# MaxHalford/sorobn

Measured on NVIDIA H100. Metric: exact-inference queries/sec, higher is better.
Workload: dtype f32

## Files before the change

### sorobn_b200/csrc/sbn_api.cu

```cuda
#include <cuda_runtime.h>

#include <algorithm>
#include <cmath>
#include <cstdarg>
#include <cstdio>
#include <cstdlib>
#include <cstring>
#include <string>
#include <vector>

#include "sbn_chain.h"
#include "sbn_count.cuh"
#include "sbn_deriv.cuh"
#include "sbn_gibbs.cuh"
#include "sbn_internal.h"
#include "sbn_join.h"
#include "sbn_kernels.cuh"
#include "sbn_launch.h"
#include "sbn_marginal.cuh"
#include "sbn_mpe.cuh"
#include "sbn_pair.h"
#include "sbn_sample.cuh"
#include "sbn_soft.cuh"
#include "sbn_tma.h"
// ... 1160 lines not shown
        sbn_soft_pack<float><<<grid, threads, 0, stream>>>(static_cast<const float *>(in.lik), in.ld_lik, rows, n_soft,
                                                           P->d_soft, P->d_arena, P->ld, P->d_log_max);
    return cudaGetLastError();
}

inline bool hoisted(const sbn_program *P, const StepDesc &st) { return P->mode == 1 && st.kind == 0; }

inline bool chain_on(const sbn_program *P) {
    return P->use_chain && P->chain_fits && P->use_tiled && !P->use_branches && !P->segments.empty();
}

inline bool pair_on(const sbn_program *P) {
    return P->use_pair && P->use_tiled && !P->use_branches && (!chain_on(P) || P->pairs_avoid_segments) && !P->pairs.empty();
}

int run_table_steps(sbn_program *P) {
    if (P->mode != 1) return SBN_OK;
    SbnStep q;
    for (const StepDesc &st : P->steps) {
        if (!hoisted(P, st)) continue;
        build_params(P, st, nullptr, 0, 1, &q);
        SBN_CUDA(launch_step(P, st, q, P->stream));
    }
    SBN_CUDA(cudaStreamSynchronize(P->stream));
    P->setup_launches = P->launches;
    P->launches = 0;
    return SBN_OK;
}

inline bool fold_normalise(const sbn_program *P, const StepDesc &st, const SbnStep &q) {
#if !SBN_FOLD_NORMALISE
    (void)P;
    (void)st;
    (void)q;
    return false;
#endif
    static const bool enabled = [] {
        const char *e = getenv("SOROBN_B200_FOLD_NORMALISE");
        return e ? atoi(e) != 0 : true;
    }();
    return enabled && P->kind == kPosterior && !P->f64 && P->post_batched && st.kind == 1 && q.tile_off != nullptr &&
           q.slab_off == nullptr && st.n_tiles == 1 && st.n_out == P->Q && !sbn_tma_eligible(P, st);
}

int issue_all(sbn_program *P, const uint8_t *d_ev, int64_t ld_ev, int64_t n_rows, float *d_out, int64_t ld_out,
              cudaStream_t stream, cudaEvent_t *events, const RunInputs &in = {}) {
    if (P->kind == kSample) SBN_CUDA(cudaMemsetAsync(in.flags(P), 0, static_cast<size_t>(n_rows), stream));
    if (!P->soft.empty()) SBN_CUDA(launch_soft_pack(P, n_rows, in, stream));
    SbnStep q;
    int k = 0;
    int n_decoded = 0;
    bool folded = false;
    bool skip_second = false;
    for (const StepDesc &st : P->steps) {
        if (events) SBN_CUDA(cudaEventRecord(events[k], stream));
        ++k;
        if (hoisted(P, st)) continue;
        if (in.forward && !P->forward[k - 1]) continue;
        if (st.kind >= 2) {
            const int decoded = st.kind == 4 || st.kind == 5 ? n_decoded++ : 0;
            SBN_CUDA(launch_kind_step(P, st, decoded, d_ev, ld_ev, n_rows, d_out, ld_out, in, stream));
            continue;
        }
        const int seg = chain_on(P) ? P->seg_first[k - 1] : -1;
        if (seg == -2) continue;
        if (seg >= 0) {
            P->launches++;
            SBN_CUDA(sbn_chain_launch(P, *P->segments[seg], d_ev, ld_ev, n_rows, d_out, ld_out, stream));
            continue;
        }
        int pair = pair_on(P) ? P->pair_first[k - 1] : -1;
        if (pair == -2 && !skip_second) pair = -1;
        skip_second = false;
        if (pair == -2) continue;
        if (pair >= 0 && !sbn_pair_fits(P, *P->pairs[pair])) pair = -1;
        if (pair >= 0) {
            skip_second = true;
            P->launches++;
            SBN_CUDA(sbn_pair_launch(P, *P->pairs[pair], d_ev, ld_ev, n_rows, stream));
            continue;
        }
        build_params(P, st, d_ev, ld_ev, n_rows, &q);
        if (k == static_cast<int>(P->steps.size()) && fold_normalise(P, st, q)) {
            q.norm_out = d_out;
            q.norm_ld = ld_out;
            q.norm_totals = P->d_total;
            q.norm_min = SBN_MIN_TOTAL_F32;
            folded = true;
        }
        SBN_CUDA(launch_step(P, st, q, stream));
    }
    if (events) SBN_CUDA(cudaEventRecord(events[k], stream));
    switch (P->kind) {
        case kPosterior:
            if (!folded && !(chain_on(P) && P->segments.back()->ends_in_posterior))
                SBN_CUDA(launch_normalise(P, d_out, ld_out, n_rows, stream));
            break;
        case kCounts:
        case kGrad: SBN_CUDA(launch_prob(P, n_rows, d_out, nullptr, stream)); break;
        case kSample: SBN_CUDA(launch_prob(P, n_rows, d_out, in.flags(P), stream)); break;
        case kJoint: SBN_CUDA(launch_prob(P, n_rows, P->d_total, nullptr, stream)); break;
        case kMarginals:
        case kMpe:
        case kMap: break;
    }
    if (events) SBN_CUDA(cudaEventRecord(events[k + 1], stream));
    return SBN_OK;
}

int issue_branched(sbn_program *P, const uint8_t *d_ev, int64_t ld_ev, int64_t n_rows, float *d_out, int64_t ld_out,
                   cudaStream_t origin, const RunInputs &in) {
    const int n_steps = static_cast<int>(P->steps.size());
    const int n_slots = static_cast<int>(P->slots.size());
    std::vector<int> last_writer(n_slots, -1);
    std::vector<std::vector<int>> readers(n_slots);
    std::vector<int> stream_of(n_steps, 0);
    cudaEvent_t fork = P->step_done[n_steps];
    if (!P->soft.empty()) SBN_CUDA(launch_soft_pack(P, n_rows, in, origin));
    SBN_CUDA(cudaEventRecord(fork, origin));
    bool joined[sbn_program::kBranches] = {false, false, false, false};
    int rr = 0;
    SbnStep q;
    for (int s = 0; s < n_steps; ++s) {
        const StepDesc &st = P->steps[s];
        if (hoisted(P, st)) continue;
        std::vector<int> deps;
        int home = -1;
        int64_t home_size = -1;
// ... 505 lines not shown
    if (n_table_floats > 0) {
        SBN_CUDA_P(cudaMalloc(&P->d_tables, static_cast<size_t>(n_table_floats) * elem));
        SBN_CUDA_P(cudaMemcpyAsync(P->d_tables, tables, static_cast<size_t>(n_table_floats) * elem,
                                   cudaMemcpyHostToDevice, P->stream));
    }
    int64_t shared_floats = 0;
    for (Slot &s : P->slots)
        if (!s.batched) shared_floats += round_up(s.padded, 64);
    if (shared_floats > 0) {
        SBN_CUDA_P(cudaMalloc(&P->d_shared, static_cast<size_t>(shared_floats) * elem));
        SBN_CUDA_P(cudaMemsetAsync(P->d_shared, 0, static_cast<size_t>(shared_floats) * elem, P->stream));
        int64_t off = 0;
        for (Slot &s : P->slots)
            if (!s.batched) {
                s.ptr = reinterpret_cast<float *>(reinterpret_cast<char *>(P->d_shared) + off * elem);
                off += round_up(s.padded, 64);
            }
    }
    {
        std::vector<int32_t> &tile_words = P->h_tile_words;
        tile_words.clear();
        plan_tiles(P, &tile_words);
        if (!tile_words.empty()) {
            SBN_CUDA_P(cudaMalloc(&P->d_tile_off, tile_words.size() * 4));
            SBN_CUDA_P(cudaMemcpyAsync(P->d_tile_off, tile_words.data(), tile_words.size() * 4,
                                       cudaMemcpyHostToDevice, P->stream));
        }
        SBN_CUDA_P(cudaStreamSynchronize(P->stream));
        if (P->kind == kPosterior && P->soft.empty()) sbn_chain_plan(P);
    }
    if (!P->soft.empty()) {
        P->use_tma = false;
        std::vector<int32_t> desc;
        for (const auto &sv : P->soft) {
            int64_t off = 0;
            for (int s = 0; s < sv.first; ++s)
                if (P->slots[s].batched) off += P->slots[s].size;
            desc.push_back(static_cast<int32_t>(off));
            desc.push_back(sv.second);
        }
        SBN_CUDA_P(cudaMalloc(&P->d_soft, desc.size() * 4));
        SBN_CUDA_P(cudaMemcpyAsync(P->d_soft, desc.data(), desc.size() * 4, cudaMemcpyHostToDevice, P->stream));
        SBN_CUDA_P(cudaStreamSynchronize(P->stream));
    }
    {
        static bool done[64] = {false};
        if (device < 64 && !done[device]) {
            SBN_CUDA_P(sbn_batched_set_attrs());
            SBN_CUDA_P(set_tiled_attrs());
            SBN_CUDA_P(sbn_chain_set_attrs());
            SBN_CUDA_P(sbn_tma_set_attrs());
            SBN_CUDA_P(sbn_join_set_attrs());
            SBN_CUDA_P(sbn_triple_rows_set_attrs());
            SBN_CUDA_P(sbn_marginal_set_attrs());
            SBN_CUDA_P(sbn_count_set_attrs());
            SBN_CUDA_P(sbn_deriv_set_attrs());
            SBN_CUDA_P(sbn_joint_set_attrs());
            SBN_CUDA_P(sbn_sample_set_attrs());
            SBN_CUDA_P(sbn_argmax_set_attrs());
            SBN_CUDA_P(sbn_batched_logdomain_set_attrs());
            done[device] = true;
        }
    }
    if (P->kind == kCounts || P->kind == kGrad) {
        for (const StepDesc &st : P->steps)
            if (st.kind == 3)
                P->partial_doubles = std::max<int64_t>(P->partial_doubles, count_grid(P, st, INT32_MAX) * SBN_COUNT_WARPS * st.span);
        SBN_CUDA_P(cudaMalloc(&P->d_counts, static_cast<size_t>(P->n_counts) * 8));
    }
#undef SBN_CUDA_P
    rc = run_table_steps(P);
    if (rc != SBN_OK) return bail(rc);
    {
        cudaError_t e = P->kind == kPosterior ? sbn_pair_plan(P) : cudaSuccess;
        if (e != cudaSuccess) return bail(fail(SBN_E_CUDA, "planning the paired steps failed: %s", cudaGetErrorString(e)));
    }
    *out = P;
    return SBN_OK;
}

int sbn_program_create(int device, const int32_t *words, int64_t n_words, const float *tables, int64_t n_table_floats,
                       sbn_program **out) {
    return create_common(device, words, n_words, tables, n_table_floats, false, out);
}

int sbn_program_create_f64(int device, const int32_t *words, int64_t n_words, const double *tables,
                           int64_t n_table_doubles, sbn_program **out) {
    return create_common(device, words, n_words, tables, n_table_doubles, true, out);
}

void sbn_program_destroy(sbn_program *P) {
    if (!P) return;
    cudaSetDevice(P->device);
    free_scratch(P);
    sbn_chain_free(P);
    sbn_pair_free(P);
    cudaFree(P->d_shared);
    cudaFree(P->d_counts);
    cudaFree(P->d_drawn);
    cudaFree(P->d_sample_args);
    cudaFree(P->d_soft);
    cudaFree(P->d_tile_off);
    cudaFree(P->d_tables);
    if (P->stream) cudaStreamDestroy(P->stream);
    for (auto &b : P->branch)
        if (b) cudaStreamDestroy(b);
// ... 757 lines not shown
```

### sorobn_b200/csrc/sbn_internal.h

```cpp
#pragma once
#include <cuda_runtime.h>
#include <stdint.h>

#include <string>
#include <utility>
#include <vector>

#include "../../include/sorobn_b200.h"

struct EvAxis {
    int col, stride, card;
};
struct InDesc {
    bool is_slot;
    int id;
    bool batched;
    int sx;
    std::vector<EvAxis> ev;
    std::vector<int> estrides;
    std::vector<int> strides;
};
struct StepDesc {
    int kind;
    int out_slot;
    int cx;
    int64_t n_out;
    std::vector<int> cards;
    std::vector<int> ecards;
    int64_t zoff_pos = -1;
    int64_t zoff_tiled_pos = -1;
    std::vector<InDesc> in;
    int tile = 0;
    int nu = 0, na = 0, nb = 0, nc = 0;
    std::vector<int> order;
    int64_t n_tiles = 0;
    int64_t tile_off_pos = 0;
    bool slab = false;
    bool big_tables = false;
    int slab_ma = 0, n_slab = 0;
    int64_t slab_off_pos = 0;
    int64_t slab_tile_off_pos = 0;
    int64_t tiles_per_super = 0, n_super = 0;
    int64_t slice_pos = -1;
    int64_t slice_tpc = 0;
    int64_t slice_smem = 0;
    int64_t q_offset = -1;
    int n_common = 0;
    std::vector<EvAxis> key;
    std::vector<int> cstrides;
    int64_t span = 0;
    int64_t soff_pos = -1, coff_pos = -1;
    bool logsumexp = false;
};
struct Slot {
    bool batched;
    int64_t size;
    int64_t padded;
    float *ptr;
};

inline int64_t round_up(int64_t v, int64_t m) { return (v + m - 1) / m * m; }
// ... 52 lines not shown
    int n_sampled = 0;
    uint8_t *d_drawn = nullptr;
    int64_t drawn_bytes = 0;
    uint32_t *d_sample_args = nullptr;
    std::vector<std::pair<int, int>> soft;
    int n_lik = 0;
    int32_t *d_soft = nullptr;
    void *d_lik = nullptr;
    double *d_log_max = nullptr;
    std::vector<char> forward;
    double *d_weight = nullptr;
    CachedGraph forward_graph;
    std::vector<std::pair<int64_t, int64_t>> tables;
    std::vector<int64_t> table_padded;
    float *d_tables = nullptr;
    std::vector<Slot> slots;
    std::vector<StepDesc> steps;

    int64_t reserved_rows = 0;
    int64_t ld = 0;
    float *d_arena = nullptr;
    float *d_shared = nullptr;
    int32_t *d_tile_off = nullptr;
    float *d_total = nullptr;
    uint8_t *d_ev = nullptr;
    float *d_out = nullptr;
    cudaStream_t stream = nullptr;
    static constexpr int kBranches = 4;
    cudaStream_t branch[kBranches] = {nullptr, nullptr, nullptr, nullptr};
    std::vector<cudaEvent_t> step_done;
    std::vector<cudaEvent_t> pipe_events;
    bool use_branches = false;

    bool use_graph = true;
    bool use_tiled = true;
    bool use_slab = true;
    bool use_preload = true;
    CachedGraph graph;
    CachedGraph pipe_graph;

    int64_t launches = 0;
    int64_t setup_launches = 0;

    std::vector<SbnSegment *> segments;
    std::vector<int> seg_first;
    float *d_chain_scratch = nullptr;
    bool use_chain = true;
    bool use_tma = true;
    bool chain_fits = true;
    std::vector<int32_t> h_tile_words;

    std::vector<SbnPair *> pairs;
    std::vector<int> pair_first;
    float *d_pair_canon = nullptr;
    int32_t *d_pair_tiles = nullptr;
    bool use_pair = true;
    bool pairs_avoid_segments = false;
};
```

### sorobn_b200/csrc/sbn_pair.cu

```cuda
#include "sbn_pair.h"

#include <algorithm>
#include <cstdlib>
#include <cstring>

#include "sbn_internal.h"
#include "sbn_kernels.cuh"
#include "sbn_launch.h"

namespace {

constexpr int kV = 2;

__device__ __forceinline__ void pair_coef8(float (&c)[SBN_PAIR_PW], const float *s) {
    const float4 lo = *reinterpret_cast<const float4 *>(s);
    const float4 hi = *reinterpret_cast<const float4 *>(s + 4);
    c[0] = lo.x, c[1] = lo.y, c[2] = lo.z, c[3] = lo.w;
    c[4] = hi.x, c[5] = hi.y, c[6] = hi.z, c[7] = hi.w;
}

template <int V>
__device__ __forceinline__ void pair_ev_offsets(const SbnPairParams &p, const SbnPairEv &d, int b, int (&e)[V]) {
#pragma unroll
    for (int l = 0; l < V; ++l) e[l] = 0;
// ... 7 lines not shown
struct PairG {
    const float *p;
    uint32_t base;
    uint32_t x[SBN_PAIR_T], d0[SBN_PAIR_T], d1[SBN_PAIR_T];
};

template <int MODE, int V>
__device__ __forceinline__ void pair_step(const float (&in)[SBN_PAIR_T][SBN_PAIR_T][V], float (&acc)[SBN_PAIR_T][SBN_PAIR_T][V],
                                          const float *k, const int (&e)[V], const PairG &G) {
    constexpr int T = SBN_PAIR_T, PW = SBN_PAIR_PW;
    constexpr bool PACKED = V == 2 && (MODE == SBN_PAIR_CE || MODE == SBN_PAIR_GB || MODE == SBN_PAIR_GC);
#pragma unroll
    for (int d0 = 0; d0 < T; ++d0)
#pragma unroll
        for (int d1 = 0; d1 < T; ++d1)
#pragma unroll
            for (int l = 0; l < V; ++l) acc[d0][d1][l] = 0.f;
#pragma unroll
    for (int x = 0; x < T; ++x) {
        float c[V][PW];
        float cp[T][V];
        if constexpr (MODE == SBN_PAIR_B) {
#pragma unroll
            for (int l = 0; l < V; ++l) pair_coef8(c[l], k + e[l] + x * PW);
        } else if constexpr (MODE == SBN_PAIR_GB) {
#pragma unroll
            for (int d1 = 0; d1 < T; ++d1) sbn_ldv<V>(cp[d1], G.p + (G.base + G.x[x] + G.d1[d1]));
        }
#pragma unroll
        for (int d0 = 0; d0 < T; ++d0) {
            if constexpr (MODE == SBN_PAIR_CU) {
                pair_coef8(c[0], k + (x * T + d0) * PW);
            } else if constexpr (MODE == SBN_PAIR_CE) {
#pragma unroll
                for (int d1 = 0; d1 < T; ++d1)
#pragma unroll
                    for (int l = 0; l < V; ++l) cp[d1][l] = k[e[l] + (x * T + d0) * T + d1];
            } else if constexpr (MODE == SBN_PAIR_GC) {
#pragma unroll
                for (int d1 = 0; d1 < T; ++d1) sbn_ldv<V>(cp[d1], G.p + (G.base + G.x[x] + G.d0[d0] + G.d1[d1]));
            }
#pragma unroll
            for (int d1 = 0; d1 < T; ++d1) {
                if constexpr (PACKED) {
                    sbn_fma2(acc[d0][d1], in[x][d0], cp[d1]);
                } else {
#pragma unroll
                    for (int l = 0; l < V; ++l)
                        acc[d0][d1][l] = fmaf(in[x][d0][l], c[MODE == SBN_PAIR_CU ? 0 : l][d1], acc[d0][d1][l]);
                }
            }
        }
    }
}

template <int M1, int M2>
__global__ void __launch_bounds__(SBN_PAIR_ROWS / kV, (M1 >= SBN_PAIR_GB ? 4 : 5)) sbn_pair_kernel(const __grid_constant__ SbnPairParams p) {
    constexpr int T = SBN_PAIR_T, V = kV;
    extern __shared__ __align__(16) float s_canon[];
    __shared__ __align__(8) uint64_t s_bar;
    sbn_pdl_launch_dependents();

    const int rblock = blockIdx.x / p.n_chunks;
    const int chunk = blockIdx.x % p.n_chunks;
    if (threadIdx.x == 0) {
        sbn_mbar_init(&s_bar, 1);
        sbn_fence_mbar_init();
    }
    __syncthreads();
    if (threadIdx.x == 0) {
        sbn_mbar_expect_tx(&s_bar, static_cast<uint32_t>(p.canon_floats) * 4u);
        sbn_tma_bulk_g2s(s_canon, p.canon, static_cast<uint32_t>(p.canon_floats) * 4u, &s_bar);
    }

    const int b = (rblock * static_cast<int>(blockDim.x) + threadIdx.x) * V;
    const bool live = b < p.n_rows;
    int e1[V], e2[V], g1[V], g2[V];
    if (live) {
        pair_ev_offsets<V>(p, p.ev_main1, b, e1);
        pair_ev_offsets<V>(p, p.ev_main2, b, e2);
        pair_ev_offsets<V>(p, p.ev_pre1, b, g1);
        pair_ev_offsets<V>(p, p.ev_pre2, b, g2);
    }
    sbn_mbar_wait(&s_bar, 0);
    if (!live) return;
    sbn_pdl_wait();

    const uint32_t ld = static_cast<uint32_t>(p.ld);
    const float *const fp = p.f + b;
    float *const op = p.out + b;
    uint32_t xs[T], ys[T], ow[T], oz[T];
#pragma unroll
    for (int d = 0; d < T; ++d) {
        xs[d] = static_cast<uint32_t>(min(d, p.cx - 1) * p.f_sx) * ld;
        ys[d] = static_cast<uint32_t>(min(d, p.cy - 1) * p.f_sy) * ld;
        ow[d] = static_cast<uint32_t>(d * p.o_sw) * ld;
        oz[d] = static_cast<uint32_t>(d * p.o_sz) * ld;
    }
    PairG G;
    G.p = p.g + b;
    G.base = 0;
    if constexpr (M1 == SBN_PAIR_GB || M1 == SBN_PAIR_GC) {
#pragma unroll
        for (int d = 0; d < T; ++d) {
            G.x[d] = static_cast<uint32_t>(d * p.g_x) * ld;
            G.d0[d] = static_cast<uint32_t>(d * p.g_y) * ld;
            G.d1[d] = static_cast<uint32_t>(d * p.g_w) * ld;
        }
    }
    const int t_begin = chunk * p.tiles_per_cta;
    const int t_end = min(p.n_tiles, t_begin + p.tiles_per_cta);

    for (int t = t_begin; t < t_end; ++t) {
        const int4 r0 = __ldg(reinterpret_cast<const int4 *>(p.tile_off) + 2 * t);
        const int4 r1 = __ldg(reinterpret_cast<const int4 *>(p.tile_off) + 2 * t + 1);
        const uint32_t ob = static_cast<uint32_t>(r0.x) * ld, fb = static_cast<uint32_t>(r0.y) * ld;

        float f[T][T][V];
#pragma unroll
        for (int x = 0; x < T; ++x)
#pragma unroll
            for (int y = 0; y < T; ++y) sbn_ldv<V>(f[x][y], fp + (fb + xs[x] + ys[y]));
        if (p.has_pre1) {
            const float *const k = s_canon + r1.x;
#pragma unroll
            for (int x = 0; x < T; ++x)
#pragma unroll
                for (int y = 0; y < T; ++y)
#pragma unroll
                    for (int l = 0; l < V; ++l) f[x][y][l] *= k[g1[l] + x * T + y];
        }
        float mid[T][T][V];
        if constexpr (M1 == SBN_PAIR_GB || M1 == SBN_PAIR_GC) G.base = static_cast<uint32_t>(r1.z) * ld;
        pair_step<M1, V>(f, mid, s_canon + r0.z, e1, G);
        if (p.has_pre2) {
            const float *const k = s_canon + r1.y;
#pragma unroll
            for (int y = 0; y < T; ++y)
#pragma unroll
                for (int w = 0; w < T; ++w)
#pragma unroll
                    for (int l = 0; l < V; ++l) mid[y][w][l] *= k[g2[l] + y * T + w];
        }
        float acc[T][T][V];
        pair_step<M2, V>(mid, acc, s_canon + r0.w, e2, G);

#pragma unroll
        for (int z = 0; z < T; ++z)
#pragma unroll
            for (int w = 0; w < T; ++w)
                if (w < p.cw && z < p.cz) sbn_stv<V>(op + (ob + ow[w] + oz[z]), acc[w][z]);
    }
}

template <int MINB>
__global__ void __launch_bounds__(SBN_TRIPLE_THREADS, MINB) sbn_triple_kernel(const __grid_constant__ SbnTripleParams p) {
    constexpr int T = SBN_PAIR_T;
    sbn_pdl_entry();
    const int rblock = blockIdx.x / p.n_chunks;
    const int chunk = blockIdx.x % p.n_chunks;
    const int b = rblock * static_cast<int>(blockDim.x) + threadIdx.x;
    if (b >= p.n_rows) return;
    const uint32_t ld = static_cast<uint32_t>(p.ld);
    const int g = threadIdx.y;
    const float *const ap = p.a + b + static_cast<uint32_t>(g * p.a_g) * ld;
    const float *const bp = p.b + b;
    const float *const cp = p.c + b;
    float *const op = p.out + b + static_cast<uint32_t>(g * p.o_g) * ld;
    uint32_t ak[T], aj[T], bj[T], bs[T], ck[T], cz[T];
#pragma unroll
    for (int d = 0; d < T; ++d) {
        ak[d] = static_cast<uint32_t>(d * p.a_k) * ld, aj[d] = static_cast<uint32_t>(d * p.a_j) * ld;
        bj[d] = static_cast<uint32_t>(d * p.b_j) * ld, bs[d] = static_cast<uint32_t>(d * p.b_s) * ld;
        ck[d] = static_cast<uint32_t>(d * p.c_k) * ld, cz[d] = static_cast<uint32_t>(d * p.c_z) * ld;
    }
    const uint32_t oz = static_cast<uint32_t>(p.o_z) * ld, os = static_cast<uint32_t>(p.o_s) * ld;
    const int t_begin = chunk * p.tiles_per_cta;
    const int t_end = min(p.n_tiles, t_begin + p.tiles_per_cta);
    for (int t = t_begin; t < t_end; ++t) {
        const int4 row = __ldg(reinterpret_cast<const int4 *>(p.tile_off) + t);
        float acc[T][T];
#pragma unroll
        for (int z = 0; z < T; ++z)
#pragma unroll
            for (int s = 0; s < T; ++s) acc[z][s] = 0.f;
#pragma unroll 1
        for (int pp = 0; pp < T; ++pp) {
            float A[T][T], B[T][T], C[T][T];
            const uint32_t a0 = static_cast<uint32_t>(row.y + pp * p.a_p) * ld, b0 = static_cast<uint32_t>(row.z + pp * p.b_p) * ld,
                           c0 = static_cast<uint32_t>(row.w + pp * p.c_p) * ld;
#pragma unroll
            for (int j = 0; j < T; ++j)
#pragma unroll
                for (int s = 0; s < T; ++s) B[j][s] = bp[b0 + bj[j] + bs[s]];
#pragma unroll
            for (int k = 0; k < T; ++k)
#pragma unroll
                for (int j = 0; j < T; ++j) A[k][j] = ap[a0 + ak[k] + aj[j]];
#pragma unroll
            for (int k = 0; k < T; ++k)
#pragma unroll
                for (int z = 0; z < T; ++z) C[k][z] = cp[c0 + ck[k] + cz[z]];
#pragma unroll
            for (int k = 0; k < T; ++k) {
                float n[T];
// ... 252 lines not shown
    for (int k = 0; k < n2; ++k)
        if (k != ks && k != kz && k != kg) r2.push_back(k), n_tiles *= s2.cards[k];
    if (n_tiles >= (1LL << 27)) return nullptr;

    SbnPair *pr = new SbnPair();
    memset(&pr->q, 0, sizeof pr->q);
    memset(&pr->t, 0, sizeof pr->t);
    pr->kind = 1;
    pr->step1 = i1, pr->step2 = i2;
    pr->g_in = -1;
    pr->a_in = ai, pr->b_in = 1 - ai, pr->c_in = 1 - mi;
    pr->tile_off_pos = static_cast<int64_t>(tiles->size());
    SbnTripleParams &q = pr->t;
    q.n_tiles = static_cast<int32_t>(n_tiles);
    q.a_j = A.estrides[0], q.a_k = A.strides[jk], q.a_p = A.strides[jp];
    q.b_j = B.estrides[0], q.b_s = B.strides[to1[ks]], q.b_p = B.strides[jp];
    q.c_k = C.estrides[kk], q.c_p = C.estrides[1 - kk], q.c_z = C.strides[kz];
    int64_t os = 1;
    std::vector<int64_t> os2(n2);
    for (int k = 0; k < n2; ++k) os2[k] = os, os *= s2.cards[k];
    q.o_z = static_cast<int32_t>(os2[kz]);
    q.o_s = static_cast<int32_t>(os2[ks]);
    q.group = kg >= 0 ? T : 1;
    q.o_g = kg >= 0 ? static_cast<int32_t>(os2[kg]) : 0;
    q.a_g = kg >= 0 ? A.strides[to1[kg]] : 0;
    std::vector<int> dig(r2.size(), 0);
    for (int64_t t = 0; t < n_tiles; ++t) {
        int64_t ob = 0, ab = 0, bb = 0, cb = 0;
        for (size_t k = 0; k < r2.size(); ++k) {
            const int ax = r2[k];
            ob += dig[k] * os2[ax];
            cb += static_cast<int64_t>(dig[k]) * C.strides[ax];
            if (to1[ax] >= 0) {
                ab += static_cast<int64_t>(dig[k]) * A.strides[to1[ax]];
                bb += static_cast<int64_t>(dig[k]) * B.strides[to1[ax]];
            }
        }
        tiles->push_back(static_cast<int32_t>(ob));
        tiles->push_back(static_cast<int32_t>(ab));
        tiles->push_back(static_cast<int32_t>(bb));
        tiles->push_back(static_cast<int32_t>(cb));
        for (size_t k = 0; k < dig.size(); ++k) {
            if (++dig[k] < s2.cards[r2[k]]) break;
            dig[k] = 0;
        }
    }
    sbn_triple_rows_plan(q, tiles->data() + pr->tile_off_pos, &pr->rows);
    return pr;
}

}

cudaError_t sbn_pair_set_attrs() {
    return cudaSuccess;
}

void sbn_pair_free(sbn_program *P) {
    for (SbnPair *pr : P->pairs) delete pr;
    P->pairs.clear();
    P->pair_first.clear();
    cudaFree(P->d_pair_canon);
    cudaFree(P->d_pair_tiles);
    P->d_pair_canon = nullptr;
    P->d_pair_tiles = nullptr;
}

cudaError_t sbn_pair_plan(sbn_program *P) {
    constexpr int T = SBN_PAIR_T;
    P->pair_first.assign(P->steps.size(), -1);
    if (P->mode != 1 || P->f64) return cudaSuccess;
    static const int min_card = [] {
        const char *e = getenv("SOROBN_B200_PAIR_MIN_CARD");
        return e ? atoi(e) : 4;
    }();

    static const bool triples_on = [] {
        const char *e = getenv("SOROBN_B200_TRIPLE");
        return e ? atoi(e) != 0 : true;
    }();

    HostTables H;
    std::vector<float> canon;
    std::vector<int32_t> tiles;
    cudaError_t err = cudaSuccess;
    bool fetched = false;

    const int n_steps = static_cast<int>(P->steps.size());
    auto launched = [&](int i) { return P->steps[i].kind != 0; };
    P->pairs_avoid_segments = P->use_chain && !P->segments.empty();
    auto in_segment = [&](int i) { return P->pairs_avoid_segments && P->seg_first[i] != -1; };
    for (int i1 = 0; i1 < n_steps; ++i1) {
        if (!launched(i1) || P->pair_first[i1] != -1) continue;
        int i2 = i1 + 1;
        while (i2 < n_steps && !launched(i2)) ++i2;
        if (i2 >= n_steps) break;
        if (in_segment(i1) || in_segment(i2)) continue;
        const StepDesc &s1 = P->steps[i1], &s2 = P->steps[i2];
        if (triples_on) {
            if (SbnPair *tr = plan_triple(P, i1, i2, &tiles)) {
                P->pair_first[i1] = static_cast<int>(P->pairs.size());
                P->pair_first[i2] = -2;
                P->pairs.push_back(tr);
                continue;
            }
        }
        if (s1.kind != 1 || s2.kind != 1 || s1.ecards.size() != 1 || s2.ecards.size() != 1) continue;
        if (s1.tile == 0 || s2.tile == 0) continue;
        int fi = -1, gi = -1, mi = -1, n_b1 = 0, n_b2 = 0;
        for (int i = 0; i < static_cast<int>(s1.in.size()); ++i)
            if (s1.in[i].batched) gi = fi, fi = i, ++n_b1;
        for (int i = 0; i < static_cast<int>(s2.in.size()); ++i)
            if (s2.in[i].batched) mi = i, ++n_b2;
        if (n_b1 < 1 || n_b1 > 2 || n_b2 != 1) continue;
        const InDesc &M = s2.in[mi];
        if (!M.is_slot || M.id != s1.out_slot || !M.ev.empty()) continue;
        if (n_b1 == 2) {
            if (s1.in.size() != 2) continue;
            const int jy0 = axis_of_stride(s1.cards, M.estrides[0]);
            if (jy0 < 0) continue;
            if (s1.in[fi].strides[jy0] == 0 || (s1.in[gi].strides[jy0] != 0 && P->slots[s1.in[gi].id].size > P->slots[s1.in[fi].id].size))
                std::swap(fi, gi);
            if (!s1.in[gi].is_slot || !s1.in[gi].ev.empty() || s1.in[gi].id == s2.out_slot) continue;
// ... 67 lines not shown
            fill_canon(g2, canon.data() + pr->canon_pos + at_g2);
            q.n_tiles = static_cast<int32_t>(n_tiles);
            q.f_sx = F.estrides[0];
            q.f_sy = F.strides[jy];
            q.cx = cx, q.cy = cy, q.cw = s2.cards[kw], q.cz = s2.cards[kz];
            int64_t os = 1;
            std::vector<int64_t> os2(n2);
            for (int k = 0; k < n2; ++k) os2[k] = os, os *= s2.cards[k];
            q.o_sw = static_cast<int32_t>(os2[kw]);
            q.o_sz = static_cast<int32_t>(os2[kz]);
            if (gi >= 0) q.g_x = s1.in[gi].estrides[0], q.g_y = s1.in[gi].strides[jy], q.g_w = s1.in[gi].strides[jw];
            q.has_pre1 = g1.tabs.empty() ? 0 : 1;
            q.has_pre2 = g2.tabs.empty() ? 0 : 1;
            set_ev(&q.ev_main1, c1);
            set_ev(&q.ev_main2, c2);
            set_ev(&q.ev_pre1, g1);
            set_ev(&q.ev_pre2, g2);
            std::vector<int> dig(r2.size(), 0);
            for (int64_t t = 0; t < n_tiles; ++t) {
                int64_t ob = 0, fb = 0;
                for (size_t k = 0; k < r2.size(); ++k) {
                    ob += dig[k] * os2[r2[k]];
                    fb += static_cast<int64_t>(dig[k]) * F.strides[r1[k]];
                }
                tiles.push_back(static_cast<int32_t>(ob));
                tiles.push_back(static_cast<int32_t>(fb));
                tiles.push_back(static_cast<int32_t>(at_c1 + tile_slab(c1, r1, dig)));
                tiles.push_back(static_cast<int32_t>(at_c2 + tile_slab(c2, r2, dig)));
                tiles.push_back(static_cast<int32_t>(at_g1 + tile_slab(g1, r1, dig)));
                tiles.push_back(static_cast<int32_t>(at_g2 + tile_slab(g2, r2, dig)));
                int64_t gb = 0;
                if (gi >= 0)
                    for (size_t k = 0; k < r1.size(); ++k) gb += static_cast<int64_t>(dig[k]) * s1.in[gi].strides[r1[k]];
                tiles.push_back(static_cast<int32_t>(gb));
                tiles.push_back(0);
                for (size_t k = 0; k < dig.size(); ++k) {
                    if (++dig[k] < s2.cards[r2[k]]) break;
                    dig[k] = 0;
                }
            }
            P->pair_first[i1] = static_cast<int>(P->pairs.size());
            P->pair_first[i2] = -2;
            P->pairs.push_back(pr);
            break;
        }
    }
    if (P->pairs.empty()) return cudaSuccess;
    err = cudaMalloc(&P->d_pair_canon, std::max<size_t>(canon.size(), 4) * 4);
    if (err != cudaSuccess) return err;
    err = cudaMalloc(&P->d_pair_tiles, tiles.size() * 4);
    if (err != cudaSuccess) return err;
    if (!canon.empty()) err = cudaMemcpy(P->d_pair_canon, canon.data(), canon.size() * 4, cudaMemcpyHostToDevice);
    if (err != cudaSuccess) return err;
    return cudaMemcpy(P->d_pair_tiles, tiles.data(), tiles.size() * 4, cudaMemcpyHostToDevice);
}

static cudaError_t triple_launch(sbn_program *P, const SbnPair &pr, int64_t n_rows, cudaStream_t stream) {
    SbnTripleParams q = pr.t;
    const StepDesc &s1 = P->steps[pr.step1], &s2 = P->steps[pr.step2];
    q.a = P->slots[s1.in[pr.a_in].id].ptr;
    q.b = P->slots[s1.in[pr.b_in].id].ptr;
    q.c = P->slots[s2.in[pr.c_in].id].ptr;
    q.out = P->slots[s2.out_slot].ptr;
    q.ld = P->ld;
    q.n_rows = static_cast<int32_t>(n_rows);
    q.tile_off = P->d_pair_tiles + pr.tile_off_pos;
    if (sbn_triple_rows_launch(P, pr.rows, q, stream)) return cudaGetLastError();
    const int rows_per_cta = q.group > 1 ? 32 : 128;
    const int64_t n_rblocks = (n_rows + rows_per_cta - 1) / rows_per_cta;
    static const int64_t tpc_env = [] {
        const char *e = getenv("SOROBN_B200_TRIPLE_TPC");
        return e ? atoll(e) : 1LL;
    }();
    static const int minb = [] {
        const char *e = getenv("SOROBN_B200_TRIPLE_MINB");
        return e ? atoi(e) : 3;
    }();
    const int64_t tpc = std::max<int64_t>(1, std::min<int64_t>(q.n_tiles, tpc_env));
    q.tiles_per_cta = static_cast<int32_t>(tpc);
    q.n_chunks = static_cast<int32_t>((q.n_tiles + tpc - 1) / tpc);
    const int64_t grid = q.n_chunks * n_rblocks;
    if (grid >= (1LL << 31)) return cudaErrorInvalidConfiguration;
    const dim3 g(static_cast<unsigned>(grid)), b(rows_per_cta, q.group);
    if (minb == 3) sbn_launch(sbn_triple_kernel<3>, g, b, 0, stream, q);
    else if (minb == 1) sbn_launch(sbn_triple_kernel<1>, g, b, 0, stream, q);
    else sbn_launch(sbn_triple_kernel<2>, g, b, 0, stream, q);
    return cudaGetLastError();
}

bool sbn_pair_fits(const sbn_program *P, const SbnPair &pr) {
    const StepDesc &s1 = P->steps[pr.step1], &s2 = P->steps[pr.step2];
    int64_t entries = P->slots[s2.out_slot].size;
    for (const InDesc &in : s1.in)
        if (in.batched) entries = std::max(entries, P->slots[in.id].size);
    for (const InDesc &in : s2.in)
        if (in.batched && in.id != s1.out_slot) entries = std::max(entries, P->slots[in.id].size);
    const char *e = getenv("SOROBN_B200_PAIR_IDX_LIMIT");
    const int64_t limit = e ? atoll(e) : (1LL << 31);
    return entries * P->ld < limit;
}

cudaError_t sbn_pair_launch(sbn_program *P, const SbnPair &pr, const uint8_t *d_ev, int64_t ld_ev, int64_t n_rows,
                            cudaStream_t stream) {
    if (pr.kind == 1) return triple_launch(P, pr, n_rows, stream);
    SbnPairParams q = pr.q;
    const StepDesc &s1 = P->steps[pr.step1], &s2 = P->steps[pr.step2];
    q.f = P->slots[s1.in[pr.f_in].id].ptr;
    q.g = pr.g_in >= 0 ? P->slots[s1.in[pr.g_in].id].ptr : q.f;
    q.out = P->slots[s2.out_slot].ptr;
    q.ev = d_ev;
    q.ld_ev = ld_ev;
    q.ld = P->ld;
    q.n_rows = static_cast<int32_t>(n_rows);
    q.canon = P->d_pair_canon + pr.canon_pos;
    q.tile_off = P->d_pair_tiles + pr.tile_off_pos;
    const int64_t n_rblocks = (n_rows + SBN_PAIR_ROWS - 1) / SBN_PAIR_ROWS;
    static const int64_t target_env = [] {
        const char *e = getenv("SOROBN_B200_PAIR_CTAS");
        return e ? atoll(e) : 0LL;
    }();
    const int64_t target = target_env > 0 ? target_env : 8LL * P->n_sms * 6;
    const int64_t chunks = std::max<int64_t>(1, std::min<int64_t>(q.n_tiles, target / std::max<int64_t>(1, n_rblocks)));
    const int64_t tpc = (q.n_tiles + chunks - 1) / chunks;
    q.tiles_per_cta = static_cast<int32_t>(tpc);
    q.n_chunks = static_cast<int32_t>((q.n_tiles + tpc - 1) / tpc);
    const int64_t grid = q.n_chunks * n_rblocks;
    if (grid >= (1LL << 31)) return cudaErrorInvalidConfiguration;
    launch_modes(pr, q, static_cast<unsigned>(grid), static_cast<size_t>(q.canon_floats) * 4, stream);
    return cudaGetLastError();
}
```

### sorobn_b200/csrc/sbn_pair.h

```cpp
#pragma once
#include <cuda_runtime.h>
#include <stdint.h>

#include <vector>

#include "../../include/sorobn_b200.h"

#define SBN_PAIR_T 5
#define SBN_PAIR_PW 8
#define SBN_PAIR_MAX_EV 4
#define SBN_PAIR_ROWS 256
#define SBN_TRIPLE_THREADS 160
#define SBN_PAIR_SMEM_MAX (40 * 1024)

struct SbnPairEv {
    int32_t n;
    int32_t col[SBN_PAIR_MAX_EV], stride[SBN_PAIR_MAX_EV], card[SBN_PAIR_MAX_EV];
};

struct SbnPairParams {
    const float *f;
    float *out;
    const uint8_t *ev;
    const float *canon;
// ... 3 lines not shown
    int32_t canon_floats;
    int32_t n_tiles, tiles_per_cta, n_chunks;
    int32_t f_sx, f_sy;
    int32_t cx, cy, cw, cz;
    int32_t o_sw, o_sz;
    int32_t has_pre1, has_pre2;
    SbnPairEv ev_main1, ev_main2, ev_pre1, ev_pre2;
    const float *g;
    int32_t g_x, g_y, g_w;
};

enum SbnPairMode { SBN_PAIR_B = 0, SBN_PAIR_CU = 1, SBN_PAIR_CE = 2, SBN_PAIR_GB = 3, SBN_PAIR_GC = 4 };

struct SbnTripleParams {
    const float *a, *b, *c;
    float *out;
    const int32_t *tile_off;
    int64_t ld;
    int32_t n_rows;
    int32_t n_tiles, tiles_per_cta, n_chunks;
    int32_t a_p, a_k, a_j;
    int32_t b_p, b_j, b_s;
    int32_t c_p, c_k, c_z;
    int32_t o_z, o_s;
    int32_t group;
    int32_t a_g, o_g;
};

#define SBN_TRIPLE_ROWS_R 16
#define SBN_TRIPLE_ROWS_COMBOS 25
#define SBN_TRIPLE_ROWS_MIN_COMBOS 8
struct SbnTripleRows {
    int ok;
    int n_combos;
    int32_t u_card[3], u_stride[3];
    int32_t u_dig[3][SBN_TRIPLE_ROWS_COMBOS];
    int32_t o_off[SBN_TRIPLE_ROWS_COMBOS];
};

struct SbnPair {
    int kind;
    int step1, step2;
    int f_in;
    int g_in;
    int m1, m2;
    SbnPairParams q;
    SbnTripleParams t;
    SbnTripleRows rows;
    int a_in, b_in, c_in;
    int64_t tile_off_pos;
    int64_t canon_pos;
};

struct sbn_program;
cudaError_t sbn_pair_plan(sbn_program *P);
cudaError_t sbn_pair_launch(sbn_program *P, const SbnPair &pr, const uint8_t *d_ev, int64_t ld_ev, int64_t n_rows,
                            cudaStream_t stream);
bool sbn_pair_fits(const sbn_program *P, const SbnPair &pr);
cudaError_t sbn_pair_set_attrs();
void sbn_pair_free(sbn_program *P);

void sbn_triple_rows_plan(const SbnTripleParams &q, const int32_t *tiles, SbnTripleRows *rows);
bool sbn_triple_rows_launch(const sbn_program *P, const SbnTripleRows &rows, const SbnTripleParams &q, cudaStream_t stream);
cudaError_t sbn_triple_rows_set_attrs();
```

Before: 25.38 million.

## Fuse chains of linked pair steps into one persistent shared-memory kernel

Adds a planner that finds consecutive pair contractions whose intermediate slot is consumed only by the next pair, and a persistent kernel that runs the whole run per 16-row block. The input rows stay in shared memory, are double-buffered with cp.async, and only the final output is written back. Canonical tables and tile offsets are loaded once with bulk TMA. The goal is to remove the global-memory round trips for intermediate slots and the separate launches. The cost is heavy shared-memory use, a per-pair runtime mode switch, and __syncthreads between pairs, which may limit occupancy.

```diff
diff --git a/sorobn_b200/csrc/sbn_api.cu b/sorobn_b200/csrc/sbn_api.cu
--- a/sorobn_b200/csrc/sbn_api.cu
+++ b/sorobn_b200/csrc/sbn_api.cu
@@ -1236,10 +1236,12 @@
     int n_decoded = 0;
     bool folded = false;
     bool skip_second = false;
+    int run_last = -1;
     for (const StepDesc &st : P->steps) {
         if (events) SBN_CUDA(cudaEventRecord(events[k], stream));
         ++k;
         if (hoisted(P, st)) continue;
+        if (k - 1 <= run_last) continue;
         if (in.forward && !P->forward[k - 1]) continue;
         if (st.kind >= 2) {
             const int decoded = st.kind == 4 || st.kind == 5 ? n_decoded++ : 0;
@@ -1258,6 +1260,13 @@
         skip_second = false;
         if (pair == -2) continue;
         if (pair >= 0 && !sbn_pair_fits(P, *P->pairs[pair])) pair = -1;
+        const int run = pair >= 0 ? sbn_pair_run_at(P, pair, n_rows) : -1;
+        if (run >= 0) {
+            run_last = P->pair_runs[run].last_step;
+            P->launches++;
+            SBN_CUDA(sbn_pair_run_launch(P, P->pair_runs[run], d_ev, ld_ev, n_rows, stream));
+            continue;
+        }
         if (pair >= 0) {
             skip_second = true;
             P->launches++;
@@ -1869,6 +1878,7 @@
             SBN_CUDA_P(sbn_tma_set_attrs());
             SBN_CUDA_P(sbn_join_set_attrs());
             SBN_CUDA_P(sbn_triple_rows_set_attrs());
+            SBN_CUDA_P(sbn_pair_set_attrs());
             SBN_CUDA_P(sbn_marginal_set_attrs());
             SBN_CUDA_P(sbn_count_set_attrs());
             SBN_CUDA_P(sbn_deriv_set_attrs());
diff --git a/sorobn_b200/csrc/sbn_internal.h b/sorobn_b200/csrc/sbn_internal.h
--- a/sorobn_b200/csrc/sbn_internal.h
+++ b/sorobn_b200/csrc/sbn_internal.h
@@ -7,6 +7,7 @@
 #include <vector>
 
 #include "../../include/sorobn_b200.h"
+#include "sbn_pair.h"
 
 struct EvAxis {
     int col, stride, card;
@@ -165,6 +166,8 @@
 
     std::vector<SbnPair *> pairs;
     std::vector<int> pair_first;
+    std::vector<SbnPairRun> pair_runs;
+    std::vector<int> pair_run_of;
     float *d_pair_canon = nullptr;
     int32_t *d_pair_tiles = nullptr;
     bool use_pair = true;
diff --git a/sorobn_b200/csrc/sbn_pair.cu b/sorobn_b200/csrc/sbn_pair.cu
--- a/sorobn_b200/csrc/sbn_pair.cu
+++ b/sorobn_b200/csrc/sbn_pair.cu
@@ -83,6 +83,63 @@
             }
         }
     }
+}
+
+struct PairIo {
+    const float *fp;
+    float *op;
+    uint32_t fb, ob;
+    uint32_t xs[SBN_PAIR_T], ys[SBN_PAIR_T];
+    uint32_t ow[SBN_PAIR_T], oz[SBN_PAIR_T];
+};
+
+template <int M1, int M2, int V, bool SHARED>
+__device__ __forceinline__ void pair_tile(const SbnPairParams &p, const float *s_canon, const int4 r0, const int4 r1,
+                                          const PairIo &io, PairG &G, uint32_t g_ld, const int (&e1)[V], const int (&e2)[V],
+                                          const int (&g1)[V], const int (&g2)[V]) {
+    constexpr int T = SBN_PAIR_T;
+    float f[T][T][V];
+#pragma unroll
+    for (int x = 0; x < T; ++x)
+#pragma unroll
+        for (int y = 0; y < T; ++y) sbn_ldv<V>(f[x][y], io.fp + (io.fb + io.xs[x] + io.ys[y]));
+    if constexpr (SHARED) __syncthreads();
+    if (p.has_pre1) {
+        const float *const k = s_canon + r1.x;
+#pragma unroll
+        for (int x = 0; x < T; ++x)
+#pragma unroll
+            for (int y = 0; y < T; ++y)
+#pragma unroll
+                for (int l = 0; l < V; ++l) f[x][y][l] *= k[g1[l] + x * T + y];
+    }
+    float mid[T][T][V];
+    if constexpr (M1 == SBN_PAIR_GB || M1 == SBN_PAIR_GC) G.base = static_cast<uint32_t>(r1.z) * g_ld;
+    pair_step<M1, V>(f, mid, s_canon + r0.z, e1, G);
+    if (p.has_pre2) {
+        const float *const k = s_canon + r1.y;
+#pragma unroll
+        for (int y = 0; y < T; ++y)
+#pragma unroll
+            for (int w = 0; w < T; ++w)
+#pragma unroll
+                for (int l = 0; l < V; ++l) mid[y][w][l] *= k[g2[l] + y * T + w];
+    }
+    float acc[T][T][V];
+    pair_step<M2, V>(mid, acc, s_canon + r0.w, e2, G);
+
+#pragma unroll
+    for (int z = 0; z < T; ++z)
+#pragma unroll
+        for (int w = 0; w < T; ++w)
+            if (w < p.cw && z < p.cz) {
+                float *const dst = io.op + (io.ob + io.ow[w] + io.oz[z]);
+                if constexpr (SHARED) {
+                    *reinterpret_cast<typename SbnVec<V>::type *>(dst) = *reinterpret_cast<const typename SbnVec<V>::type *>(acc[w][z]);
+                } else {
+                    sbn_stv<V>(dst, acc[w][z]);
+                }
+            }
 }
 
 template <int M1, int M2>
@@ -118,15 +175,15 @@
     sbn_pdl_wait();
 
     const uint32_t ld = static_cast<uint32_t>(p.ld);
-    const float *const fp = p.f + b;
-    float *const op = p.out + b;
-    uint32_t xs[T], ys[T], ow[T], oz[T];
+    PairIo io;
+    io.fp = p.f + b;
+    io.op = p.out + b;
 #pragma unroll
     for (int d = 0; d < T; ++d) {
-        xs[d] = static_cast<uint32_t>(min(d, p.cx - 1) * p.f_sx) * ld;
-        ys[d] = static_cast<uint32_t>(min(d, p.cy - 1) * p.f_sy) * ld;
-        ow[d] = static_cast<uint32_t>(d * p.o_sw) * ld;
-        oz[d] = static_cast<uint32_t>(d * p.o_sz) * ld;
+        io.xs[d] = static_cast<uint32_t>(min(d, p.cx - 1) * p.f_sx) * ld;
+        io.ys[d] = static_cast<uint32_t>(min(d, p.cy - 1) * p.f_sy) * ld;
+        io.ow[d] = static_cast<uint32_t>(d * p.o_sw) * ld;
+        io.oz[d] = static_cast<uint32_t>(d * p.o_sz) * ld;
     }
     PairG G;
     G.p = p.g + b;
@@ -145,43 +202,133 @@
     for (int t = t_begin; t < t_end; ++t) {
         const int4 r0 = __ldg(reinterpret_cast<const int4 *>(p.tile_off) + 2 * t);
         const int4 r1 = __ldg(reinterpret_cast<const int4 *>(p.tile_off) + 2 * t + 1);
-        const uint32_t ob = static_cast<uint32_t>(r0.x) * ld, fb = static_cast<uint32_t>(r0.y) * ld;
-
-        float f[T][T][V];
-#pragma unroll
-        for (int x = 0; x < T; ++x)
-#pragma unroll
-            for (int y = 0; y < T; ++y) sbn_ldv<V>(f[x][y], fp + (fb + xs[x] + ys[y]));
-        if (p.has_pre1) {
-            const float *const k = s_canon + r1.x;
-#pragma unroll
-            for (int x = 0; x < T; ++x)
-#pragma unroll
-                for (int y = 0; y < T; ++y)
-#pragma unroll
-                    for (int l = 0; l < V; ++l) f[x][y][l] *= k[g1[l] + x * T + y];
-        }
-        float mid[T][T][V];
-        if constexpr (M1 == SBN_PAIR_GB || M1 == SBN_PAIR_GC) G.base = static_cast<uint32_t>(r1.z) * ld;
-        pair_step<M1, V>(f, mid, s_canon + r0.z, e1, G);
-        if (p.has_pre2) {
-            const float *const k = s_canon + r1.y;
-#pragma unroll
-            for (int y = 0; y < T; ++y)
-#pragma unroll
-                for (int w = 0; w < T; ++w)
-#pragma unroll
-                    for (int l = 0; l < V; ++l) mid[y][w][l] *= k[g2[l] + y * T + w];
-        }
-        float acc[T][T][V];
-        pair_step<M2, V>(mid, acc, s_canon + r0.w, e2, G);
-
-#pragma unroll
-        for (int z = 0; z < T; ++z)
-#pragma unroll
-            for (int w = 0; w < T; ++w)
-                if (w < p.cw && z < p.cz) sbn_stv<V>(op + (ob + ow[w] + oz[z]), acc[w][z]);
-    }
+        io.ob = static_cast<uint32_t>(r0.x) * ld, io.fb = static_cast<uint32_t>(r0.y) * ld;
+        pair_tile<M1, M2, V, false>(p, s_canon, r0, r1, io, G, ld, e1, e2, g1, g2);
+    }
+}
+
+struct SbnPairRunParams {
+    SbnPairParams q[SBN_PAIR_RUN_MAX];
+    int32_t mode[SBN_PAIR_RUN_MAX];
+    int32_t canon_off[SBN_PAIR_RUN_MAX];
+    int32_t tile_off[SBN_PAIR_RUN_MAX];
+    const int32_t *tiles;
+    int32_t tile_words;
+    const float *f;
+    float *out;
+    const float *canon;
+    int64_t ld;
+    int32_t n_pairs, n_rows, n_blocks;
+    int32_t canon_floats;
+    int32_t entries;
+    int32_t f_entries, out_entries;
+};
+
+__device__ __forceinline__ void cp_async16(float *dst, const float *src) {
+    asm volatile("cp.async.cg.shared.global [%0], [%1], 16;" ::"r"(sbn_smem_u32(dst)), "l"(src) : "memory");
+}
+
+__global__ void __launch_bounds__(SBN_PAIR_RUN_THREADS, 2) sbn_pair_run_kernel(const __grid_constant__ SbnPairRunParams p) {
+    constexpr int T = SBN_PAIR_T, V = kV, R = SBN_PAIR_RUN_R;
+    extern __shared__ __align__(16) float s_mem[];
+    __shared__ __align__(8) uint64_t s_bar;
+    float *const s_canon = s_mem + 2 * p.entries * R;
+    int32_t *const s_tiles = reinterpret_cast<int32_t *>(s_canon + p.canon_floats);
+    int32_t *const s_ev = s_tiles + p.tile_words;
+    sbn_pdl_launch_dependents();
+    if (threadIdx.x == 0) {
+        sbn_mbar_init(&s_bar, 1);
+        sbn_fence_mbar_init();
+    }
+    __syncthreads();
+    if (threadIdx.x == 0) {
+        sbn_mbar_expect_tx(&s_bar, static_cast<uint32_t>(p.canon_floats + p.tile_words) * 4u);
+        sbn_tma_bulk_g2s(s_canon, p.canon, static_cast<uint32_t>(p.canon_floats) * 4u, &s_bar);
+        sbn_tma_bulk_g2s(s_tiles, p.tiles, static_cast<uint32_t>(p.tile_words) * 4u, &s_bar);
+    }
+    const int rt = static_cast<int>(threadIdx.x) % (R / V);
+    const int t = static_cast<int>(threadIdx.x) / (R / V);
+    sbn_mbar_wait(&s_bar, 0);
+    sbn_pdl_wait();
+
+    const uint32_t ld = static_cast<uint32_t>(p.ld);
+    const int n_vec = R / 4;
+    auto fetch = [&](int blk, float *buf) {
+        if (blk < p.n_blocks)
+            for (int i = threadIdx.x; i < p.f_entries * n_vec; i += blockDim.x) {
+                const int en = i / n_vec, v = i % n_vec;
+                cp_async16(buf + en * R + 4 * v, p.f + (static_cast<uint32_t>(en) * ld + blk * R + 4 * v));
+            }
+        asm volatile("cp.async.commit_group;" ::: "memory");
+    };
+    fetch(blockIdx.x, s_mem);
+    int cur = 0;
+    for (int blk = blockIdx.x; blk < p.n_blocks; blk += gridDim.x, cur ^= 1) {
+        const int row0 = blk * R;
+        float *const s_front = s_mem + cur * p.entries * R;
+        fetch(blk + gridDim.x, s_mem + (cur ^ 1) * p.entries * R);
+        for (int i = threadIdx.x; i < p.n_pairs * 4 * R; i += blockDim.x) {
+            const int j = i / (4 * R), a = (i / R) % 4, r = i % R;
+            const SbnPairParams &q = p.q[j];
+            const SbnPairEv &d = a == 0 ? q.ev_main1 : a == 1 ? q.ev_main2 : a == 2 ? q.ev_pre1 : q.ev_pre2;
+            int e = 0;
+            for (int k = 0; k < d.n; ++k)
+                e += ((row0 + r < p.n_rows) ? min(static_cast<int>(q.ev[static_cast<int64_t>(d.col[k]) * q.ld_ev + row0 + r]), d.card[k] - 1) : 0) *
+                     d.stride[k];
+            s_ev[i] = e;
+        }
+        asm volatile("cp.async.wait_group 1;" ::: "memory");
+        __syncthreads();
+
+        for (int j = 0; j < p.n_pairs; ++j) {
+            const SbnPairParams &q = p.q[j];
+            int e1[V], e2[V], g1[V], g2[V];
+            const int32_t *const ev = s_ev + j * 4 * R + rt * V;
+#pragma unroll
+            for (int l = 0; l < V; ++l) e1[l] = ev[l], e2[l] = ev[R + l], g1[l] = ev[2 * R + l], g2[l] = ev[3 * R + l];
+            const int4 r0 = reinterpret_cast<const int4 *>(s_tiles + p.tile_off[j])[2 * t];
+            const int4 r1 = reinterpret_cast<const int4 *>(s_tiles + p.tile_off[j])[2 * t + 1];
+            PairIo io;
+            io.fp = s_front + rt * V;
+            io.op = s_front + rt * V;
+            io.fb = static_cast<uint32_t>(r0.y) * R, io.ob = static_cast<uint32_t>(r0.x) * R;
+#pragma unroll
+            for (int d = 0; d < T; ++d) {
+                io.xs[d] = static_cast<uint32_t>(min(d, q.cx - 1) * q.f_sx) * R;
+                io.ys[d] = static_cast<uint32_t>(min(d, q.cy - 1) * q.f_sy) * R;
+                io.ow[d] = static_cast<uint32_t>(d * q.o_sw) * R;
+                io.oz[d] = static_cast<uint32_t>(d * q.o_sz) * R;
+            }
+            PairG G;
+            const float *const k = s_canon + p.canon_off[j];
+#define SBN_PAIR_RUN_CASE(A, B)                                                  \
+    case A * 3 + B:                                                              \
+        pair_tile<A, B, V, true>(q, k, r0, r1, io, G, ld, e1, e2, g1, g2);       \
+        break;
+            switch (p.mode[j]) {
+                SBN_PAIR_RUN_CASE(0, 0)
+                SBN_PAIR_RUN_CASE(0, 1)
+                SBN_PAIR_RUN_CASE(0, 2)
+                SBN_PAIR_RUN_CASE(1, 0)
+                SBN_PAIR_RUN_CASE(1, 1)
+                SBN_PAIR_RUN_CASE(1, 2)
+                SBN_PAIR_RUN_CASE(2, 0)
+                SBN_PAIR_RUN_CASE(2, 1)
+                SBN_PAIR_RUN_CASE(2, 2)
+            }
+#undef SBN_PAIR_RUN_CASE
+            __syncthreads();
+        }
+
+        for (int i = threadIdx.x; i < p.out_entries * n_vec; i += blockDim.x) {
+            const int en = i / n_vec, v = i % n_vec;
+            if (row0 + 4 * v < p.n_rows)
+                __stcs(reinterpret_cast<float4 *>(p.out + (static_cast<uint32_t>(en) * ld + row0 + 4 * v)),
+                       *reinterpret_cast<const float4 *>(s_front + en * R + 4 * v));
+        }
+        __syncthreads();
+    }
+    asm volatile("cp.async.wait_all;" ::: "memory");
 }
 
 template <int MINB>
@@ -540,22 +687,110 @@
 }
 
 cudaError_t sbn_pair_set_attrs() {
-    return cudaSuccess;
+    return cudaFuncSetAttribute(sbn_pair_run_kernel, cudaFuncAttributeMaxDynamicSharedMemorySize, SBN_PAIR_RUN_SMEM_MAX);
 }
 
 void sbn_pair_free(sbn_program *P) {
     for (SbnPair *pr : P->pairs) delete pr;
     P->pairs.clear();
     P->pair_first.clear();
+    P->pair_runs.clear();
+    P->pair_run_of.clear();
     cudaFree(P->d_pair_canon);
     cudaFree(P->d_pair_tiles);
     P->d_pair_canon = nullptr;
     P->d_pair_tiles = nullptr;
 }
 
+static void pair_extents(const sbn_program *P, const SbnPair &pr, const std::vector<int32_t> &tiles, int64_t *f, int64_t *o) {
+    const SbnPairParams &q = pr.q;
+    int64_t f_hi = 0, o_hi = 0;
+    for (int t = 0; t < q.n_tiles; ++t) {
+        const int32_t *row = tiles.data() + pr.tile_off_pos + 8 * t;
+        f_hi = std::max<int64_t>(f_hi, row[1] + static_cast<int64_t>(q.cx - 1) * q.f_sx + static_cast<int64_t>(q.cy - 1) * q.f_sy);
+        o_hi = std::max<int64_t>(o_hi, row[0] + static_cast<int64_t>(q.cw - 1) * q.o_sw + static_cast<int64_t>(q.cz - 1) * q.o_sz);
+    }
+    const int64_t n_out = P->steps[pr.step2].n_out;
+    *f = f_hi + 1;
+    *o = static_cast<int64_t>(q.n_tiles) * q.cw * q.cz == n_out && o_hi + 1 == n_out ? n_out : 0;
+}
+
+static int64_t run_smem(int64_t entries, int64_t canon_floats, int64_t tile_words, int n_pairs) {
+    return (2 * entries * SBN_PAIR_RUN_R + canon_floats + tile_words + static_cast<int64_t>(n_pairs) * 4 * SBN_PAIR_RUN_R) * 4;
+}
+
+static cudaError_t plan_runs(sbn_program *P, const std::vector<int32_t> &tiles) {
+    constexpr int R = SBN_PAIR_RUN_R, V = kV;
+    P->pair_runs.clear();
+    P->pair_run_of.assign(P->pairs.size(), -1);
+    const int n_steps = static_cast<int>(P->steps.size()), n_pairs = static_cast<int>(P->pairs.size());
+    std::vector<int64_t> f_ext(n_pairs, 0), o_ext(n_pairs, 0);
+    auto covered = [&](int j) {
+        const SbnPair &pr = *P->pairs[j];
+        if (pr.kind != 0 || pr.g_in >= 0 || pr.q.n_tiles * (R / V) > SBN_PAIR_RUN_THREADS) return false;
+        pair_extents(P, pr, tiles, &f_ext[j], &o_ext[j]);
+        return o_ext[j] > 0;
+    };
+    auto linked = [&](int a, int b) {
+        const SbnPair &pa = *P->pairs[a], &pb = *P->pairs[b];
+        int next = pa.step2 + 1;
+        while (next < n_steps && P->steps[next].kind == 0) ++next;
+        if (pb.step1 != next || pa.q.n_tiles != pb.q.n_tiles) return false;
+        const int slot = P->steps[pa.step2].out_slot;
+        const StepDesc &s1 = P->steps[pb.step1];
+        if (slot == P->post_slot || !s1.in[pb.f_in].is_slot || s1.in[pb.f_in].id != slot) return false;
+        if (pb.canon_pos != pa.canon_pos + pa.q.canon_floats || pb.tile_off_pos != pa.tile_off_pos + 8LL * pa.q.n_tiles) return false;
+        for (int i = pb.step1; i < n_steps; ++i) {
+            const StepDesc &st = P->steps[i];
+            for (int k = 0; k < static_cast<int>(st.in.size()); ++k)
+                if (st.in[k].is_slot && st.in[k].id == slot && !(i == pb.step1 && k == pb.f_in)) return false;
+            if (st.out_slot == slot) break;
+        }
+        return f_ext[b] <= o_ext[a];
+    };
+    auto smem = [&](int first, int n) {
+        int64_t entries = f_ext[first], canon = 0, words = 0;
+        for (int j = first; j < first + n; ++j)
+            entries = std::max(entries, o_ext[j]), canon += P->pairs[j]->q.canon_floats, words += 8LL * P->pairs[j]->q.n_tiles;
+        return run_smem(entries, canon, words, n);
+    };
+    for (int j = 0; j < n_pairs;) {
+        if (!covered(j)) {
+            ++j;
+            continue;
+        }
+        int n = 1;
+        while (j + n < n_pairs && n < SBN_PAIR_RUN_MAX && covered(j + n) && linked(j + n - 1, j + n) &&
+               smem(j, n + 1) <= SBN_PAIR_RUN_SMEM_MAX)
+            ++n;
+        if (n >= 2 && smem(j, n) <= SBN_PAIR_RUN_SMEM_MAX) {
+            SbnPairRun run;
+            run.first = j, run.n = n;
+            run.last_step = P->pairs[j + n - 1]->step2;
+            run.entries = static_cast<int>(f_ext[j]);
+            run.f_entries = static_cast<int>(f_ext[j]);
+            run.out_entries = static_cast<int>(o_ext[j + n - 1]);
+            run.canon_floats = 0;
+            for (int k = j; k < j + n; ++k) run.entries = std::max<int>(run.entries, static_cast<int>(o_ext[k])), run.canon_floats += P->pairs[k]->q.canon_floats;
+            const int threads = P->pairs[j]->q.n_tiles * (R / V);
+            cudaError_t err = cudaOccupancyMaxActiveBlocksPerMultiprocessor(&run.blocks_per_sm, sbn_pair_run_kernel, threads,
+                                                                            static_cast<size_t>(smem(j, n)));
+            if (err != cudaSuccess) return err;
+            if (run.blocks_per_sm > 0) {
+                P->pair_run_of[j] = static_cast<int>(P->pair_runs.size());
+                P->pair_runs.push_back(run);
+            }
+        }
+        j += n;
+    }
+    return cudaSuccess;
+}
+
 cudaError_t sbn_pair_plan(sbn_program *P) {
     constexpr int T = SBN_PAIR_T;
     P->pair_first.assign(P->steps.size(), -1);
+    P->pair_runs.clear();
+    P->pair_run_of.clear();
     if (P->mode != 1 || P->f64) return cudaSuccess;
     static const int min_card = [] {
         const char *e = getenv("SOROBN_B200_PAIR_MIN_CARD");
@@ -729,7 +964,9 @@
     if (err != cudaSuccess) return err;
     if (!canon.empty()) err = cudaMemcpy(P->d_pair_canon, canon.data(), canon.size() * 4, cudaMemcpyHostToDevice);
     if (err != cudaSuccess) return err;
-    return cudaMemcpy(P->d_pair_tiles, tiles.data(), tiles.size() * 4, cudaMemcpyHostToDevice);
+    err = cudaMemcpy(P->d_pair_tiles, tiles.data(), tiles.size() * 4, cudaMemcpyHostToDevice);
+    if (err != cudaSuccess) return err;
+    return plan_runs(P, tiles);
 }
 
 static cudaError_t triple_launch(sbn_program *P, const SbnPair &pr, int64_t n_rows, cudaStream_t stream) {
@@ -777,9 +1014,7 @@
     return entries * P->ld < limit;
 }
 
-cudaError_t sbn_pair_launch(sbn_program *P, const SbnPair &pr, const uint8_t *d_ev, int64_t ld_ev, int64_t n_rows,
-                            cudaStream_t stream) {
-    if (pr.kind == 1) return triple_launch(P, pr, n_rows, stream);
+static SbnPairParams pair_params(const sbn_program *P, const SbnPair &pr, const uint8_t *d_ev, int64_t ld_ev, int64_t n_rows) {
     SbnPairParams q = pr.q;
     const StepDesc &s1 = P->steps[pr.step1], &s2 = P->steps[pr.step2];
     q.f = P->slots[s1.in[pr.f_in].id].ptr;
@@ -791,6 +1026,60 @@
     q.n_rows = static_cast<int32_t>(n_rows);
     q.canon = P->d_pair_canon + pr.canon_pos;
     q.tile_off = P->d_pair_tiles + pr.tile_off_pos;
+    return q;
+}
+
+int sbn_pair_run_at(const sbn_program *P, int pair, int64_t n_rows) {
+    if (pair < 0 || pair >= static_cast<int>(P->pair_run_of.size()) || P->pair_run_of[pair] < 0) return -1;
+    if (n_rows < 2LL * P->n_sms * 32) return -1;
+    const char *e = getenv("SOROBN_B200_PAIR_RUNS");
+    if (e && atoi(e) == 0) return -1;
+    const SbnPairRun &run = P->pair_runs[P->pair_run_of[pair]];
+    for (int j = run.first; j < run.first + run.n; ++j)
+        if (!sbn_pair_fits(P, *P->pairs[j])) return -1;
+    return P->pair_run_of[pair];
+}
+
+cudaError_t sbn_pair_run_launch(sbn_program *P, const SbnPairRun &run, const uint8_t *d_ev, int64_t ld_ev, int64_t n_rows,
+                                cudaStream_t stream) {
+    constexpr int R = SBN_PAIR_RUN_R;
+    SbnPairRunParams p;
+    memset(&p, 0, sizeof p);
+    int64_t canon_off = 0, tile_off = 0;
+    for (int j = 0; j < run.n; ++j) {
+        const SbnPair &pr = *P->pairs[run.first + j];
+        p.q[j] = pair_params(P, pr, d_ev, ld_ev, n_rows);
+        p.mode[j] = pr.m1 * 3 + pr.m2;
+        p.canon_off[j] = static_cast<int32_t>(canon_off);
+        p.tile_off[j] = static_cast<int32_t>(tile_off);
+        canon_off += pr.q.canon_floats;
+        tile_off += 8LL * pr.q.n_tiles;
+    }
+    p.tiles = p.q[0].tile_off;
+    p.tile_words = static_cast<int32_t>(tile_off);
+    p.f = p.q[0].f;
+    p.out = p.q[run.n - 1].out;
+    p.canon = p.q[0].canon;
+    p.ld = P->ld;
+    p.n_pairs = run.n;
+    p.n_rows = static_cast<int32_t>(n_rows);
+    const int64_t n_blocks = (n_rows + R - 1) / R;
+    p.n_blocks = static_cast<int32_t>(n_blocks);
+    p.canon_floats = static_cast<int32_t>(run.canon_floats);
+    p.entries = run.entries;
+    p.f_entries = run.f_entries;
+    p.out_entries = run.out_entries;
+    const int threads = P->pairs[run.first]->q.n_tiles * (R / kV);
+    const int64_t grid = std::min<int64_t>(n_blocks, static_cast<int64_t>(P->n_sms) * run.blocks_per_sm);
+    const size_t smem = static_cast<size_t>(run_smem(run.entries, run.canon_floats, tile_off, run.n));
+    sbn_launch(sbn_pair_run_kernel, dim3(static_cast<unsigned>(grid)), dim3(threads), smem, stream, p);
+    return cudaGetLastError();
+}
+
+cudaError_t sbn_pair_launch(sbn_program *P, const SbnPair &pr, const uint8_t *d_ev, int64_t ld_ev, int64_t n_rows,
+                            cudaStream_t stream) {
+    if (pr.kind == 1) return triple_launch(P, pr, n_rows, stream);
+    SbnPairParams q = pair_params(P, pr, d_ev, ld_ev, n_rows);
     const int64_t n_rblocks = (n_rows + SBN_PAIR_ROWS - 1) / SBN_PAIR_ROWS;
     static const int64_t target_env = [] {
         const char *e = getenv("SOROBN_B200_PAIR_CTAS");
diff --git a/sorobn_b200/csrc/sbn_pair.h b/sorobn_b200/csrc/sbn_pair.h
--- a/sorobn_b200/csrc/sbn_pair.h
+++ b/sorobn_b200/csrc/sbn_pair.h
@@ -79,6 +79,20 @@
     int64_t canon_pos;
 };
 
+#define SBN_PAIR_RUN_R 16
+#define SBN_PAIR_RUN_MAX 4
+#define SBN_PAIR_RUN_THREADS 224
+#define SBN_PAIR_RUN_SMEM_MAX (226 * 1024)
+
+struct SbnPairRun {
+    int first, n;
+    int last_step;
+    int entries;
+    int f_entries, out_entries;
+    int64_t canon_floats;
+    int blocks_per_sm;
+};
+
 struct sbn_program;
 cudaError_t sbn_pair_plan(sbn_program *P);
 cudaError_t sbn_pair_launch(sbn_program *P, const SbnPair &pr, const uint8_t *d_ev, int64_t ld_ev, int64_t n_rows,
@@ -86,6 +100,9 @@
 bool sbn_pair_fits(const sbn_program *P, const SbnPair &pr);
 cudaError_t sbn_pair_set_attrs();
 void sbn_pair_free(sbn_program *P);
+int sbn_pair_run_at(const sbn_program *P, int pair, int64_t n_rows);
+cudaError_t sbn_pair_run_launch(sbn_program *P, const SbnPairRun &run, const uint8_t *d_ev, int64_t ld_ev, int64_t n_rows,
+                                cudaStream_t stream);
 
 void sbn_triple_rows_plan(const SbnTripleParams &q, const int32_t *tiles, SbnTripleRows *rows);
 bool sbn_triple_rows_launch(const sbn_program *P, const SbnTripleRows &rows, const SbnTripleParams &q, cudaStream_t stream);
```

Result: faster. 27.14 million (median of 6 runs) (+6.9%).
